# cover-vla/cover-vla

Hardware: AMD Instinct MI355X
Metric: candidate actions scored/sec (whole node), OpenVLA-7B N=32, 224^2 RGB (higher is better)
Workload: dtype bf16; 1 GPU; OpenVLA-7B (DINOv2-L+SigLIP-So400m+Llama-2-7B) N=32 = 8 prompts x 4 samples per GPU, 7 action tokens, 1 224x224 RGB frame(s); CoVer verifier SigLIP2-L/16-384 + 3-member ensemble; random-init weights with decision margins (depth-scaled residual projections, unit-scale embeddings, log-normal gains on the action rows of the head: synth.openvla_state(peaked=True)); candidates_total=32, candidates_per_gpu=32, prompts_per_gpu=8, parallelism=candidate-sharded x1 (weak), own_kv=legacy

## Files before the change

cover_vla_amd/csrc/decode_attn.hip:

```cpp
#include "common.h"
#include "kernels.h"

struct DecAttnDev {
    const bf16_t* qkv; int ld_qkv;
    const float* partial; int n_splits; const float* bias;
    int N, H;
    float scale_log2e;
    const int* positions; const float* cos_t; const float* sin_t; int n_pos, rope_mode;
    const bf16_t* k0; const bf16_t* vt0; int k0_t, k0_h, vt0_h, vt0_d, len0;
    const bf16_t* k1; const bf16_t* vt1; long long k1_slot, vt1_slot; int k1_t, k1_h, vt1_h, vt1_d; const int* slot1; const int* len1; int len1_c;
    bf16_t* k2; bf16_t* vt2; long long k2_slot, vt2_slot; int k2_t, k2_h, vt2_h, vt2_d; const int* slot2; int len2, write_t;
    bf16_t* out; long long o_row;
    int WA, WC;
    int tail_tile;
};

constexpr int DA_NW = 16;

#ifdef COVER_DA_DEBUG
__device__ unsigned long long g_da_dbg[512 * 8];
extern "C" int cover_da_debug(unsigned long long* out) { return (int)hipMemcpyFromSymbol(out, HIP_SYMBOL(g_da_dbg), sizeof(g_da_dbg)); }
#define DAT(slot) do { if (threadIdx.x == 0) g_da_dbg[(((blockIdx.z * gridDim.y + blockIdx.y) * gridDim.x + blockIdx.x) & 511) * 8 + (slot)] = wall_clock64(); } while (0)
__device__ unsigned long long g_da_wave[16 * 8];
extern "C" int cover_da_debug_waves(unsigned long long* out) { return (int)hipMemcpyFromSymbol(out, HIP_SYMBOL(g_da_wave), sizeof(g_da_wave)); }
#define DAW(slot, val) do { if ((threadIdx.x & 63) == 0 && blockIdx.x == 1 && blockIdx.y == 7 && blockIdx.z == 2) g_da_wave[(threadIdx.x >> 6) * 8 + (slot)] = (val); } while (0)
#else
#define DAT(slot) do { } while (0)
#define DAW(slot, val) do { } while (0)
#endif
template <int D, int VS>
__global__ __launch_bounds__(1024) void decode_attn_fused_k(DecAttnDev a) {
    DAT(0);
    DAW(6, wall_clock64());
    constexpr int KS = D / 32, DB = D / 16 / VS, HALF = D / 2, DV = D / VS;
    constexpr int OW = DB * 4 * 64;
    constexpr int IPW = (DB * 4 + DA_NW - 1) / DA_NW;
    static_assert(DB * 4 % DA_NW == 0 || DB * 4 < DA_NW, "merge items must split evenly over the waves");
    __shared__ __attribute__((aligned(16))) bf16_t qs[16 * D];
    __shared__ __attribute__((aligned(16))) bf16_t kn[16 * D];
    __shared__ __attribute__((aligned(16))) bf16_t vn[16 * D];
    __shared__ float so[(DA_NW + 1) * OW];
    __shared__ float sm[(DA_NW + 1) * 16];
    __shared__ float sl[(DA_NW + 1) * 16];
    const int tid = threadIdx.x, lane = tid & 63;
    const int w = __builtin_amdgcn_readfirstlane(tid >> 6);
    const int tile = blockIdx.x, h = blockIdx.y;
    const int dv0 = blockIdx.z * DV;
    const int r = lane & 15, g = lane >> 4;
    const int ncols = 3 * a.H * D;
    const int WB = DA_NW - a.WA - a.WC;

    const int cand_r = tile * 16 + r;
    const bool q_ok = cand_r < a.N;
    const int my_slot1 = q_ok ? (a.slot1 ? a.slot1[cand_r] : cand_r) : -1;
    const int my_len1 = q_ok ? (a.len1 ? a.len1[cand_r] : a.len1_c) : 0;
    const bool p1 = tid < 16 * HALF;
    const int pc = tid / HALF, pi = tid - pc * HALF;
    const int pcand = tile * 16 + pc;
    const bool p1_ok = p1 && pcand < a.N;
    int ppos = 0, pslot2 = pcand;
    if (p1_ok) {
        if (a.rope_mode != 0) ppos = a.positions[pcand];
        if (a.slot2) pslot2 = a.slot2[pcand];
    }
#ifdef COVER_DA_DEBUG
    asm volatile("s_waitcnt vmcnt(0)" ::: "memory");
#endif
    DAT(4);
    float x[6] = {0.f, 0.f, 0.f, 0.f, 0.f, 0.f};
    float cs = 1.f, sn = 0.f;
    if (p1_ok) {
        unsigned col[6];
#pragma unroll
        for (int j = 0; j < 3; ++j) {
            col[2 * j] = (unsigned)((j * a.H + h) * D + pi);
            col[2 * j + 1] = col[2 * j] + HALF;
        }
        float pv[6][4], bs[6] = {0.f, 0.f, 0.f, 0.f, 0.f, 0.f};
        const unsigned pstride = (unsigned)a.N * (unsigned)ncols;
        if (a.n_splits <= 0) {
            const unsigned ro = (unsigned)pcand * (unsigned)a.ld_qkv;
#pragma unroll
            for (int j = 0; j < 6; ++j) x[j] = bf2f(a.qkv[ro + col[j]]);
        } else {
            const unsigned ro = (unsigned)pcand * (unsigned)ncols;
#pragma unroll
            for (int sidx = 0; sidx < 4; ++sidx) {
                if (sidx < a.n_splits) {
                    const float* ps = a.partial + (size_t)sidx * pstride;
#pragma unroll
                    for (int j = 0; j < 6; ++j) pv[j][sidx] = ps[ro + col[j]];
                } else {
#pragma unroll
                    for (int j = 0; j < 6; ++j) pv[j][sidx] = 0.f;
                }
            }
            if (a.bias) {
#pragma unroll
                for (int j = 0; j < 6; ++j) bs[j] = a.bias[col[j]];
            }
        }
        if (a.rope_mode != 0) {
            ppos = ppos < 0 ? 0 : (ppos >= a.n_pos ? a.n_pos - 1 : ppos);
            const unsigned po = (unsigned)(ppos * HALF + pi);
            cs = a.cos_t[po];
            sn = a.sin_t[po];
        }
        if (a.n_splits > 0) {
            const unsigned ro = (unsigned)pcand * (unsigned)ncols;
#pragma unroll
            for (int j = 0; j < 6; ++j) {
                float v = 0.f;
#pragma unroll
                for (int sidx = 0; sidx < 4; ++sidx) v += sidx < a.n_splits ? pv[j][sidx] : 0.f;
                for (int sidx = 4; sidx < a.n_splits; ++sidx) v += a.partial[(size_t)sidx * pstride + ro + col[j]];
                if (a.bias) v += bs[j];
                x[j] = bfround(v);
            }
        }
    }

    asm volatile("s_waitcnt vmcnt(0)" ::: "memory");
    DAT(5);
    bool leader = q_ok;
#pragma unroll
    for (int j = 0; j < 15; ++j) {
        const int other = __shfl(my_slot1, (lane & 48) | j);
        leader = leader && !(j < r && other == my_slot1);
    }
    const unsigned leaders = (unsigned)(__ballot(leader && g == 0) & 0xffffull);
    const int role = w < a.WA ? 0 : (w < a.WA + WB ? 1 : 2);
    const int wl = role == 0 ? w : (role == 1 ? w - a.WA : w - a.WA - WB);
    const int cl = 4 * wl;

    const bf16_t* kbase = nullptr;
    const bf16_t* vbase = nullptr;
    unsigned ko0 = 0, ko1 = 0;
    unsigned vo = 0;
    unsigned vstep = 0;
    unsigned vmask = 0;
    int it = -1, bcol = -1, bslot = 0, blen = 0;
    bool tail_pending = (VS >= 2 && role == 2 && wl == 0 && a.tail_tile >= 0), is_tail = false;
    auto next_tile = [&]() -> bool {
        if (role == 0) {
            it = it < 0 ? wl : it + a.WA;
            const int t0 = 32 * it;
            if (t0 >= a.len0 || it == a.tail_tile) return false;
            int key0 = t0 + 8 * (r >> 2) + (r & 3), key1 = key0 + 4;
            key0 = key0 < a.len0 ? key0 : a.len0 - 1;
            key1 = key1 < a.len0 ? key1 : a.len0 - 1;
            kbase = a.k0 + h * a.k0_h;
            ko0 = key0 * a.k0_t + g * 8;
            ko1 = key1 * a.k0_t + g * 8;
            vbase = a.vt0 + h * a.vt0_h + t0;
            vo = r * a.vt0_d + g * 8;
            vstep = 16 * a.vt0_d;
            vmask = 0;
#pragma unroll
            for (int e = 0; e < 8; ++e) vmask |= (q_ok && t0 + 8 * g + e < a.len0) ? (1u << e) : 0u;
            return true;
        }
        if (role == 1) {
            ++it;
            if (bcol < 0 || 32 * it >= blen) {
                it = 0;
                bool found = false;
                for (int c = bcol + 1; c < 16 && !found; ++c) {
                    if (!((leaders >> c) & 1u)) continue;
                    if (__popc(leaders & ((1u << c) - 1u)) % WB != wl) continue;
                    const int glen = __shfl(my_len1, c);
                    if (glen <= 0) continue;
                    bcol = c; bslot = __builtin_amdgcn_readfirstlane(__shfl(my_slot1, c)); blen = __builtin_amdgcn_readfirstlane(glen);
                    found = true;
                }
                if (!found) return false;
            }
            const int t0 = 32 * it;
            int key0 = t0 + 8 * (r >> 2) + (r & 3), key1 = key0 + 4;
            key0 = key0 < blen ? key0 : blen - 1;
            key1 = key1 < blen ? key1 : blen - 1;
            kbase = a.k1 + (long long)bslot * a.k1_slot + h * a.k1_h;
            ko0 = key0 * a.k1_t + g * 8;
            ko1 = key1 * a.k1_t + g * 8;
            vbase = a.vt1 + (long long)bslot * a.vt1_slot + h * a.vt1_h + t0;
            vo = r * a.vt1_d + g * 8;
            vstep = 16 * a.vt1_d;
            vmask = 0;
#pragma unroll
            for (int e = 0; e < 8; ++e) vmask |= (q_ok && my_slot1 == bslot && t0 + 8 * g + e < blen) ? (1u << e) : 0u;
            return true;
        }
        ++it;
        const int tb = 8 * it;
        if (tb >= a.len2) {
            if (VS < 2 || !tail_pending) return false;
            tail_pending = false;
            is_tail = true;
            const int t0 = 32 * a.tail_tile;
            int key0 = t0 + 8 * (r >> 2) + (r & 3), key1 = key0 + 4;
            key0 = key0 < a.len0 ? key0 : a.len0 - 1;
            key1 = key1 < a.len0 ? key1 : a.len0 - 1;
            kbase = a.k0 + h * a.k0_h;
            ko0 = key0 * a.k0_t + g * 8;
            ko1 = key1 * a.k0_t + g * 8;
            vbase = a.vt0 + h * a.vt0_h + t0;
            vo = r * a.vt0_d + g * 8;
            vstep = 16 * a.vt0_d;
            vmask = 0;
#pragma unroll
            for (int e = 0; e < 8; ++e) vmask |= (q_ok && t0 + 8 * g + e < a.len0) ? (1u << e) : 0u;
            return true;
        }
        int cg = tile * 16 + cl + (r >> 2), cv = tile * 16 + cl + g;
        cg = cg < a.N ? cg : a.N - 1;
        cv = cv < a.N ? cv : a.N - 1;
        const int sk = a.slot2 ? a.slot2[cg] : cg, sv = a.slot2 ? a.slot2[cv] : cv;
        int ta = tb + (r & 3), tc = ta + 4;
        ta = ta < a.len2 ? ta : a.len2 - 1;
        tc = tc < a.len2 ? tc : a.len2 - 1;
        kbase = a.k2 + h * a.k2_h;
        ko0 = (unsigned)sk * (unsigned)a.k2_slot + ta * a.k2_t + g * 8;
        ko1 = (unsigned)sk * (unsigned)a.k2_slot + tc * a.k2_t + g * 8;
        vbase = a.vt2 + h * a.vt2_h + tb;
        vo = (unsigned)sv * (unsigned)a.vt2_slot + r * a.vt2_d;
        vstep = 16 * a.vt2_d;
        vmask = 0;
#pragma unroll
        for (int e = 0; e < 8; ++e) vmask |= (q_ok && cl + g == r && tb + e < a.len2) ? (1u << e) : 0u;
        return true;
    };
    u32x4 kr0[KS], kr1[KS], vr[DB];
    auto load_tile = [&]() {
#pragma unroll
        for (int ks = 0; ks < KS; ++ks) {
            kr0[ks] = *(const u32x4*)(kbase + ko0 + ks * 32);
            kr1[ks] = *(const u32x4*)(kbase + ko1 + ks * 32);
        }
#pragma unroll
        for (int db = 0; db < DB; ++db) vr[db] = *(const u32x4*)(vbase + vo + (db + (dv0 >> 4)) * vstep);
    };
    if (p1) {
        if (p1_ok) {
            if (a.rope_mode == 2) {
                cs = bfround(cs); sn = bfround(sn);
                const float a1 = bfround(bfround(x[0] * cs) + bfround(-x[1] * sn)), a2 = bfround(bfround(x[1] * cs) + bfround(x[0] * sn));
                const float b1 = bfround(bfround(x[2] * cs) + bfround(-x[3] * sn)), b2 = bfround(bfround(x[3] * cs) + bfround(x[2] * sn));
                x[0] = a1; x[1] = a2; x[2] = b1; x[3] = b2;
            } else if (a.rope_mode != 0) {
#pragma clang fp contract(off)
                const float a1 = x[0] * cs - x[1] * sn, a2 = x[1] * cs + x[0] * sn;
                const float b1 = x[2] * cs - x[3] * sn, b2 = x[3] * cs + x[2] * sn;
                x[0] = a1; x[1] = a2; x[2] = b1; x[3] = b2;
            }
        }
        qs[pc * D + pi] = f2bf(x[0]);
        qs[pc * D + pi + HALF] = f2bf(x[1]);
        kn[pc * D + pi] = f2bf(x[2]);
        kn[pc * D + pi + HALF] = f2bf(x[3]);
        vn[pc * D + pi] = f2bf(x[4]);
        vn[pc * D + pi + HALF] = f2bf(x[5]);
    }
    DAT(6);
    bool have = next_tile();
    if (have) load_tile();
    DAW(0, wall_clock64());
    DAW(4, (unsigned long long)role);
    asm volatile("s_waitcnt lgkmcnt(0)\n\ts_barrier" ::: "memory");
    DAT(1);
    DAW(1, wall_clock64());
    if (p1_ok) {
        bf16_t* kd = a.k2 + a.write_t * a.k2_t + h * a.k2_h;
        const unsigned kof = (unsigned)pslot2 * (unsigned)a.k2_slot + pi;
        if (blockIdx.z == 0) { kd[kof] = f2bf(x[2]); kd[kof + HALF] = f2bf(x[3]); }
        bf16_t* vd = a.vt2 + h * a.vt2_h + a.write_t;
        const unsigned vof = (unsigned)pslot2 * (unsigned)a.vt2_slot + pi * a.vt2_d;
        if (pi >= dv0 && pi < dv0 + DV) vd[vof] = f2bf(x[4]);
        if (pi + HALF >= dv0 && pi + HALF < dv0 + DV) vd[vof + HALF * a.vt2_d] = f2bf(x[5]);
    }

    bool first = true;
#ifdef COVER_DA_DEBUG
    int dbg_tiles = 0;
#endif
    int sw = w;
#pragma clang loop unroll(disable)
    while (have) {
        if (VS >= 2 && is_tail && sw == w) {
            if (first) {
#pragma unroll
                for (int i = 0; i < DB * 4; ++i) so[w * OW + i * 64 + lane] = 0.f;
                if (g == 0) {
                    sm[w * 16 + r] = -INFINITY;
                    sl[w * 16 + r] = 0.f;
                }
            }
            sw = DA_NW;
            first = true;
        }
        if (role == 2 && !is_tail) {
            const int e = a.write_t - 8 * it;
            if (e >= 0 && e < 8) {
                const bf16_t* kp = kn + (cl + (r >> 2)) * D + g * 8;
                const bool mine = (r & 3) == (e & 3);
#pragma unroll
                for (int ks = 0; ks < KS; ++ks) {
                    const u32x4 nk = *(const u32x4*)(kp + ks * 32);
                    kr0[ks] = (mine && e < 4) ? nk : kr0[ks];
                    kr1[ks] = (mine && e >= 4) ? nk : kr1[ks];
                    asm volatile("" ::: "memory");
                }
                const unsigned keep = (e & 1) ? 0x0000ffffu : 0xffff0000u;
                const int sh = (e & 1) ? 16 : 0, wi = e >> 1;
#pragma unroll
                for (int db = 0; db < DB; ++db) {
                    const unsigned nv = (unsigned)vn[(cl + g) * D + dv0 + db * 16 + r] << sh;
#pragma unroll
                    for (int q = 0; q < 4; ++q) vr[db][q] = (q == wi) ? ((vr[db][q] & keep) | nv) : vr[db][q];
                    asm volatile("" ::: "memory");
                }
            }
        }
        f32x4 s0 = (f32x4){0.f, 0.f, 0.f, 0.f}, s1 = s0;
#pragma unroll
        for (int ks = 0; ks < KS; ++ks) {
            const bf16x8 qf = as_bf16x8(*(const uint4*)(qs + r * D + ks * 32 + g * 8));
            s0 = __builtin_amdgcn_mfma_f32_16x16x32_bf16(__builtin_bit_cast(bf16x8, kr0[ks]), qf, s0, 0, 0, 0);
            s1 = __builtin_amdgcn_mfma_f32_16x16x32_bf16(__builtin_bit_cast(bf16x8, kr1[ks]), qf, s1, 0, 0, 0);
        }
        float sc[8], m = -INFINITY;
#pragma unroll
        for (int e = 0; e < 8; ++e) {
            sc[e] = ((vmask >> e) & 1u) ? (e < 4 ? s0[e] : s1[e - 4]) * a.scale_log2e : -INFINITY;
            m = fmaxf(m, sc[e]);
        }
        m = fmaxf(m, __shfl_xor(m, 16));
        m = fmaxf(m, __shfl_xor(m, 32));
        float l = 0.f, p[8];
#pragma unroll
        for (int e = 0; e < 8; ++e) {
            p[e] = (m == -INFINITY) ? 0.f : exp2f(sc[e] - m);
            l += p[e];
        }
        l += __shfl_xor(l, 16);
        l += __shfl_xor(l, 32);
        uint4 pp;
        pp.x = pack_bf2(p[0], p[1]); pp.y = pack_bf2(p[2], p[3]); pp.z = pack_bf2(p[4], p[5]); pp.w = pack_bf2(p[6], p[7]);
        const bf16x8 pf = as_bf16x8(pp);
        float* slot = so + sw * OW + lane;
        float fo = 0.f, ft = 1.f;
        if (!first) {
            const float mo = sm[sw * 16 + r], lo = sl[sw * 16 + r];
            const float mx = fmaxf(mo, m);
            fo = (mo == -INFINITY) ? 0.f : exp2f(mo - mx);
            ft = (m == -INFINITY) ? 0.f : exp2f(m - mx);
            m = mx;
            l = lo * fo + l * ft;
        }
#pragma unroll
        for (int db = 0; db < DB; ++db) {
            const f32x4 o = __builtin_amdgcn_mfma_f32_16x16x32_bf16(__builtin_bit_cast(bf16x8, vr[db]), pf, (f32x4){0.f, 0.f, 0.f, 0.f}, 0, 0, 0);
#pragma unroll
            for (int e = 0; e < 4; ++e) {
                float* sp = slot + (db * 4 + e) * 64;
                *sp = first ? o[e] : *sp * fo + o[e] * ft;
            }
            asm volatile("" ::: "memory");
        }
        if (g == 0) {
            sm[sw * 16 + r] = m;
            sl[sw * 16 + r] = l;
        }
#ifdef COVER_DA_DEBUG
        if (first) DAW(2, wall_clock64());
        dbg_tiles++;
#endif
        first = false;
        have = next_tile();
        if (have) load_tile();
    }
#ifdef COVER_DA_DEBUG
    DAW(3, wall_clock64());
    DAW(5, (unsigned long long)dbg_tiles);
#endif
    if (first && sw == w) {
#pragma unroll
        for (int i = 0; i < DB * 4; ++i) so[w * OW + i * 64 + lane] = 0.f;
        if (g == 0) {
            sm[w * 16 + r] = -INFINITY;
            sl[w * 16 + r] = 0.f;
        }
    }
    if (role == 2 && wl == 0 && sw == w) {
#pragma unroll
        for (int i = 0; i < DB * 4; ++i) so[DA_NW * OW + i * 64 + lane] = 0.f;
        if (g == 0) {
            sm[DA_NW * 16 + r] = -INFINITY;
            sl[DA_NW * 16 + r] = 0.f;
        }
    }

    asm volatile("s_waitcnt lgkmcnt(0)\n\ts_barrier" ::: "memory");
    DAT(2);
    if (!q_ok) return;
    float mx = -INFINITY;
#pragma unroll
    for (int i = 0; i < DA_NW + 1; ++i) mx = fmaxf(mx, sm[i * 16 + r]);
    float lt = 0.f, f[DA_NW + 1];
#pragma unroll
    for (int i = 0; i < DA_NW + 1; ++i) {
        const float mi = sm[i * 16 + r];
        f[i] = (mi == -INFINITY) ? 0.f : exp2f(mi - mx);
        lt += sl[i * 16 + r] * f[i];
    }
    const float inv = lt > 0.f ? 1.f / lt : 0.f;
    const int item0 = w * IPW, db = item0 >> 2, e0 = item0 & 3;
    if (item0 >= DB * 4) return;
    float o[IPW];
#pragma unroll
    for (int e = 0; e < IPW; ++e) {
        float acc = 0.f;
#pragma unroll
        for (int i = 0; i < DA_NW + 1; ++i) acc += so[i * OW + (item0 + e) * 64 + lane] * f[i];
        o[e] = acc * inv;
    }
    bf16_t* op = a.out + (long long)cand_r * a.o_row + (long long)h * D + dv0 + db * 16 + 4 * g + e0;
    if constexpr (IPW == 2) {
        *(uint32_t*)op = pack_bf2(o[0], o[1]);
    } else {
        *op = f2bf(o[0]);
    }
    DAT(3);
}

hipError_t launch_decode_attention_fused(const cover_decode_attn_args* x, hipStream_t st) {
    if (x->N <= 0) return hipSuccess;
    if (x->D != 64 && x->D != 128) return hipErrorInvalidValue;
    for (int i = 0; i < 3; ++i)
        if (x->seg[i].mask_mode != COVER_MASK_LEN) return hipErrorInvalidValue;
    if (x->seg[0].len <= 0 || x->seg[2].len <= 0 || x->write_t < 0 || x->write_t >= x->seg[2].len) return hipErrorInvalidValue;
    if (x->rope_mode != 0 && (!x->cos_table || !x->sin_table || !x->positions)) return hipErrorInvalidValue;
    DecAttnDev a;
    a.qkv = (const bf16_t*)x->qkv; a.ld_qkv = x->ld_qkv;
    a.partial = x->partial; a.n_splits = x->n_splits; a.bias = x->bias;
    a.N = x->N; a.H = x->H;
    a.scale_log2e = x->scale * 1.4426950408889634f;
    a.positions = x->positions; a.cos_t = x->cos_table; a.sin_t = x->sin_table; a.n_pos = x->n_pos; a.rope_mode = x->rope_mode;
    const cover_kv_segment &s0 = x->seg[0], &s1 = x->seg[1], &s2 = x->seg[2];
    const long long slot0 = 0;
    a.k0 = (const bf16_t*)s0.k + slot0 * s0.k_slot_stride; a.vt0 = (const bf16_t*)s0.vt + slot0 * s0.vt_slot_stride;
    const long long strides[] = {s0.k_t_stride, s0.k_h_stride, s0.vt_h_stride, s0.vt_d_stride, s1.k_t_stride, s1.k_h_stride, s1.vt_h_stride,
                                 s1.vt_d_stride, s2.k_t_stride, s2.k_h_stride, s2.vt_h_stride, s2.vt_d_stride};
    for (long long v : strides)
        if (v < 0 || v > (1ll << 26)) return hipErrorInvalidValue;
    if ((long long)x->N * 3 * x->H * x->D * (x->n_splits > 0 ? x->n_splits : 1) >= (1ll << 31)) return hipErrorInvalidValue;
    if (!s2.slot_of_batch && ((long long)x->N * s2.k_slot_stride >= (1ll << 31) || (long long)x->N * s2.vt_slot_stride >= (1ll << 31)))
        return hipErrorInvalidValue;
    if ((s2.vt_d_stride & 7) || (s0.vt_d_stride & 7) || (s1.vt_d_stride & 7)) return hipErrorInvalidValue;
    a.k0_t = (int)s0.k_t_stride; a.k0_h = (int)s0.k_h_stride; a.vt0_h = (int)s0.vt_h_stride; a.vt0_d = (int)s0.vt_d_stride; a.len0 = s0.len;
    a.k1 = (const bf16_t*)s1.k; a.vt1 = (const bf16_t*)s1.vt;
    a.k1_slot = s1.k_slot_stride; a.k1_t = (int)s1.k_t_stride; a.k1_h = (int)s1.k_h_stride;
    a.vt1_slot = s1.vt_slot_stride; a.vt1_h = (int)s1.vt_h_stride; a.vt1_d = (int)s1.vt_d_stride;
    a.slot1 = s1.slot_of_batch; a.len1 = s1.len_of_batch; a.len1_c = s1.len;
    a.k2 = (bf16_t*)s2.k; a.vt2 = (bf16_t*)s2.vt;
    a.k2_slot = s2.k_slot_stride; a.k2_t = (int)s2.k_t_stride; a.k2_h = (int)s2.k_h_stride;
    a.vt2_slot = s2.vt_slot_stride; a.vt2_h = (int)s2.vt_h_stride; a.vt2_d = (int)s2.vt_d_stride;
    a.slot2 = s2.slot_of_batch; a.len2 = s2.len; a.write_t = x->write_t;
    a.out = (bf16_t*)x->out; a.o_row = x->out_row_stride;
    const int nA = (s0.len + 31) / 32;
    a.WC = 4;
    a.WA = nA < 9 ? nA : 9;
    a.tail_tile = -1;
    static const char* vs_env = getenv("COVER_DA_VSPLIT");
    const int units = ((x->N + 15) / 16) * x->H;
    int VS = vs_env ? (atoi(vs_env) == 4 ? 4 : atoi(vs_env) == 2 ? 2 : 1) : (units <= 64 ? 4 : units <= 128 ? 2 : 1);
    if (x->D != 128 && VS == 4) VS = 2;
    static const char* tail_env = getenv("COVER_DA_TAIL");
    if (nA == 9 && VS >= 2 && !(tail_env && tail_env[0] == '0')) { a.WA = 8; a.tail_tile = 8; }
    dim3 grid((x->N + 15) / 16, x->H, VS), block(64 * DA_NW);
    const int pid = prof_enabled() ? prof_open(st, 2, 0.0) : -1;
    if (x->D == 128) {
        if (VS == 4) hipLaunchKernelGGL((decode_attn_fused_k<128, 4>), grid, block, 0, st, a);
        else if (VS == 2) hipLaunchKernelGGL((decode_attn_fused_k<128, 2>), grid, block, 0, st, a);
        else hipLaunchKernelGGL((decode_attn_fused_k<128, 1>), grid, block, 0, st, a);
    } else {
        if (VS == 2) hipLaunchKernelGGL((decode_attn_fused_k<64, 2>), grid, block, 0, st, a);
        else hipLaunchKernelGGL((decode_attn_fused_k<64, 1>), grid, block, 0, st, a);
    }
    prof_close(st, pid);
    return hipGetLastError();
}
```

Measured before the change: 956.8 candidates/s.

## Move decode-attn QKV prologue onto C-role waves with vector loads and priority

The QKV prologue (sum split-K partials, add bias, apply RoPE, stage q/k/v into LDS and write the new K/V to cache) now runs on the four C-role waves, each lane handling several contiguous elements with vectorized float4/uint2 loads and stores. Before, every thread in the first half of the block did one scalar element. Those waves also raise their scheduling priority until the barrier, so the prologue that gates the barrier finishes sooner while the other waves prefetch their K/V tiles. An optional late-prefetch variant is compiled in but off. The wide path needs pointer and stride alignment checks, falls back otherwise, and doubles the template instantiations.

```diff
diff --git a/cover_vla_amd/csrc/decode_attn.hip b/cover_vla_amd/csrc/decode_attn.hip
--- a/cover_vla_amd/csrc/decode_attn.hip
+++ b/cover_vla_amd/csrc/decode_attn.hip
@@ -20,19 +20,45 @@
 #ifdef COVER_DA_DEBUG
 __device__ unsigned long long g_da_dbg[512 * 8];
 extern "C" int cover_da_debug(unsigned long long* out) { return (int)hipMemcpyFromSymbol(out, HIP_SYMBOL(g_da_dbg), sizeof(g_da_dbg)); }
-#define DAT(slot) do { if (threadIdx.x == 0) g_da_dbg[(((blockIdx.z * gridDim.y + blockIdx.y) * gridDim.x + blockIdx.x) & 511) * 8 + (slot)] = wall_clock64(); } while (0)
+#define DAT_IF(cond, slot) do { if (cond) g_da_dbg[(((blockIdx.z * gridDim.y + blockIdx.y) * gridDim.x + blockIdx.x) & 511) * 8 + (slot)] = wall_clock64(); } while (0)
+#define DAT(slot) DAT_IF(threadIdx.x == 0, slot)
 __device__ unsigned long long g_da_wave[16 * 8];
 extern "C" int cover_da_debug_waves(unsigned long long* out) { return (int)hipMemcpyFromSymbol(out, HIP_SYMBOL(g_da_wave), sizeof(g_da_wave)); }
 #define DAW(slot, val) do { if ((threadIdx.x & 63) == 0 && blockIdx.x == 1 && blockIdx.y == 7 && blockIdx.z == 2) g_da_wave[(threadIdx.x >> 6) * 8 + (slot)] = (val); } while (0)
 #else
+#define DAT_IF(cond, slot) do { } while (0)
 #define DAT(slot) do { } while (0)
 #define DAW(slot, val) do { } while (0)
 #endif
-template <int D, int VS>
+#ifndef COVER_DA_P1_PRIO
+#define COVER_DA_P1_PRIO 1
+#endif
+#ifndef COVER_DA_AB_LATE
+#define COVER_DA_AB_LATE 0
+#endif
+
+template <int n> __device__ __forceinline__ void ld_f32(const float* p, float (&o)[n]) {
+    if constexpr (n == 4) { const float4 v = *(const float4*)p; o[0] = v.x; o[1] = v.y; o[2] = v.z; o[3] = v.w; }
+    else if constexpr (n == 2) { const float2 v = *(const float2*)p; o[0] = v.x; o[1] = v.y; }
+    else o[0] = *p;
+}
+template <int n> __device__ __forceinline__ void ld_bf16(const bf16_t* p, bf16_t (&o)[n]) {
+    if constexpr (n == 4) { const uint2 v = *(const uint2*)p; o[0] = (bf16_t)v.x; o[1] = (bf16_t)(v.x >> 16); o[2] = (bf16_t)v.y; o[3] = (bf16_t)(v.y >> 16); }
+    else if constexpr (n == 2) { const uint32_t v = *(const uint32_t*)p; o[0] = (bf16_t)v; o[1] = (bf16_t)(v >> 16); }
+    else o[0] = *p;
+}
+template <int n> __device__ __forceinline__ void st_bf16(bf16_t* p, const float (&x)[n]) {
+    if constexpr (n == 4) { uint2 v; v.x = pack_bf2(x[0], x[1]); v.y = pack_bf2(x[2], x[3]); *(uint2*)p = v; }
+    else if constexpr (n == 2) *(uint32_t*)p = pack_bf2(x[0], x[1]);
+    else *p = f2bf(x[0]);
+}
+
+template <int D, int VS, bool P1V>
 __global__ __launch_bounds__(1024) void decode_attn_fused_k(DecAttnDev a) {
     DAT(0);
     DAW(6, wall_clock64());
     constexpr int KS = D / 32, DB = D / 16 / VS, HALF = D / 2, DV = D / VS;
+    constexpr int PPL = P1V ? HALF / 16 : 1;
     constexpr int OW = DB * 4 * 64;
     constexpr int IPW = (DB * 4 + DA_NW - 1) / DA_NW;
     static_assert(DB * 4 % DA_NW == 0 || DB * 4 < DA_NW, "merge items must split evenly over the waves");
@@ -54,8 +80,17 @@
     const bool q_ok = cand_r < a.N;
     const int my_slot1 = q_ok ? (a.slot1 ? a.slot1[cand_r] : cand_r) : -1;
     const int my_len1 = q_ok ? (a.len1 ? a.len1[cand_r] : a.len1_c) : 0;
-    const bool p1 = tid < 16 * HALF;
-    const int pc = tid / HALF, pi = tid - pc * HALF;
+    const int role = w < a.WA ? 0 : (w < a.WA + WB ? 1 : 2);
+    const int wl = role == 0 ? w : (role == 1 ? w - a.WA : w - a.WA - WB);
+    const int cl = 4 * wl;
+#if COVER_DA_P1_PRIO
+    if constexpr (P1V) {
+        if (role == 2) __builtin_amdgcn_s_setprio(3);
+    }
+#endif
+    const bool p1 = P1V ? role == 2 : tid < 16 * HALF;
+    const int pc = P1V ? cl + g : tid / HALF, pi = P1V ? r * PPL : tid - pc * HALF;
+    const bool p1_stamp = P1V ? (role == 2 && wl == 0 && lane == 0) : tid == 0;
     const int pcand = tile * 16 + pc;
     const bool p1_ok = p1 && pcand < a.N;
     int ppos = 0, pslot2 = pcand;
@@ -66,9 +101,15 @@
 #ifdef COVER_DA_DEBUG
     asm volatile("s_waitcnt vmcnt(0)" ::: "memory");
 #endif
-    DAT(4);
-    float x[6] = {0.f, 0.f, 0.f, 0.f, 0.f, 0.f};
-    float cs = 1.f, sn = 0.f;
+    DAT_IF(p1_stamp, 4);
+    float x[6][PPL];
+    float cs[PPL], sn[PPL];
+#pragma unroll
+    for (int e = 0; e < PPL; ++e) {
+#pragma unroll
+        for (int j = 0; j < 6; ++j) x[j][e] = 0.f;
+        cs[e] = 1.f; sn[e] = 0.f;
+    }
     if (p1_ok) {
         unsigned col[6];
 #pragma unroll
@@ -76,52 +117,83 @@
             col[2 * j] = (unsigned)((j * a.H + h) * D + pi);
             col[2 * j + 1] = col[2 * j] + HALF;
         }
-        float pv[6][4], bs[6] = {0.f, 0.f, 0.f, 0.f, 0.f, 0.f};
         const unsigned pstride = (unsigned)a.N * (unsigned)ncols;
+        auto load_cos_sin = [&]() {
+            if (a.rope_mode != 0) {
+                ppos = ppos < 0 ? 0 : (ppos >= a.n_pos ? a.n_pos - 1 : ppos);
+                const unsigned po = (unsigned)(ppos * HALF + pi);
+                ld_f32<PPL>(a.cos_t + po, cs);
+                ld_f32<PPL>(a.sin_t + po, sn);
+            }
+        };
         if (a.n_splits <= 0) {
             const unsigned ro = (unsigned)pcand * (unsigned)a.ld_qkv;
 #pragma unroll
-            for (int j = 0; j < 6; ++j) x[j] = bf2f(a.qkv[ro + col[j]]);
+            for (int j = 0; j < 6; ++j) {
+                bf16_t raw[PPL];
+                ld_bf16<PPL>(a.qkv + ro + col[j], raw);
+#pragma unroll
+                for (int e = 0; e < PPL; ++e) x[j][e] = bf2f(raw[e]);
+            }
+            load_cos_sin();
         } else {
             const unsigned ro = (unsigned)pcand * (unsigned)ncols;
-#pragma unroll
-            for (int sidx = 0; sidx < 4; ++sidx) {
+            constexpr int NSL = PPL == 4 ? 2 : 4;
+            float pv[6][NSL][PPL], bs[6][PPL];
+#pragma unroll
+            for (int sidx = 0; sidx < NSL; ++sidx) {
                 if (sidx < a.n_splits) {
                     const float* ps = a.partial + (size_t)sidx * pstride;
 #pragma unroll
-                    for (int j = 0; j < 6; ++j) pv[j][sidx] = ps[ro + col[j]];
+                    for (int j = 0; j < 6; ++j) ld_f32<PPL>(ps + ro + col[j], pv[j][sidx]);
                 } else {
 #pragma unroll
-                    for (int j = 0; j < 6; ++j) pv[j][sidx] = 0.f;
-                }
-            }
-            if (a.bias) {
-#pragma unroll
-                for (int j = 0; j < 6; ++j) bs[j] = a.bias[col[j]];
-            }
-        }
-        if (a.rope_mode != 0) {
-            ppos = ppos < 0 ? 0 : (ppos >= a.n_pos ? a.n_pos - 1 : ppos);
-            const unsigned po = (unsigned)(ppos * HALF + pi);
-            cs = a.cos_t[po];
-            sn = a.sin_t[po];
-        }
-        if (a.n_splits > 0) {
-            const unsigned ro = (unsigned)pcand * (unsigned)ncols;
+                    for (int j = 0; j < 6; ++j)
+#pragma unroll
+                        for (int e = 0; e < PPL; ++e) pv[j][sidx][e] = 0.f;
+                }
+            }
 #pragma unroll
             for (int j = 0; j < 6; ++j) {
-                float v = 0.f;
-#pragma unroll
-                for (int sidx = 0; sidx < 4; ++sidx) v += sidx < a.n_splits ? pv[j][sidx] : 0.f;
-                for (int sidx = 4; sidx < a.n_splits; ++sidx) v += a.partial[(size_t)sidx * pstride + ro + col[j]];
-                if (a.bias) v += bs[j];
-                x[j] = bfround(v);
-            }
+                if (a.bias) {
+                    ld_f32<PPL>(a.bias + col[j], bs[j]);
+                } else {
+#pragma unroll
+                    for (int e = 0; e < PPL; ++e) bs[j][e] = 0.f;
+                }
+            }
+            load_cos_sin();
+            float v[6][PPL];
+#pragma unroll
+            for (int j = 0; j < 6; ++j)
+#pragma unroll
+                for (int e = 0; e < PPL; ++e) {
+                    v[j][e] = 0.f;
+#pragma unroll
+                    for (int sidx = 0; sidx < NSL; ++sidx) v[j][e] += sidx < a.n_splits ? pv[j][sidx][e] : 0.f;
+                }
+            for (int sidx = NSL; sidx < a.n_splits; ++sidx) {
+                const float* ps = a.partial + (size_t)sidx * pstride;
+                float t[6][PPL];
+#pragma unroll
+                for (int j = 0; j < 6; ++j) ld_f32<PPL>(ps + ro + col[j], t[j]);
+#pragma unroll
+                for (int j = 0; j < 6; ++j)
+#pragma unroll
+                    for (int e = 0; e < PPL; ++e) v[j][e] += t[j][e];
+            }
+#pragma unroll
+            for (int j = 0; j < 6; ++j)
+#pragma unroll
+                for (int e = 0; e < PPL; ++e) {
+                    if (a.bias) v[j][e] += bs[j][e];
+                    x[j][e] = bfround(v[j][e]);
+                }
         }
     }
 
     asm volatile("s_waitcnt vmcnt(0)" ::: "memory");
-    DAT(5);
+    DAT_IF(p1_stamp, 5);
     bool leader = q_ok;
 #pragma unroll
     for (int j = 0; j < 15; ++j) {
@@ -129,9 +201,6 @@
         leader = leader && !(j < r && other == my_slot1);
     }
     const unsigned leaders = (unsigned)(__ballot(leader && g == 0) & 0xffffull);
-    const int role = w < a.WA ? 0 : (w < a.WA + WB ? 1 : 2);
-    const int wl = role == 0 ? w : (role == 1 ? w - a.WA : w - a.WA - WB);
-    const int cl = 4 * wl;
 
     const bf16_t* kbase = nullptr;
     const bf16_t* vbase = nullptr;
@@ -242,40 +311,63 @@
     if (p1) {
         if (p1_ok) {
             if (a.rope_mode == 2) {
-                cs = bfround(cs); sn = bfround(sn);
-                const float a1 = bfround(bfround(x[0] * cs) + bfround(-x[1] * sn)), a2 = bfround(bfround(x[1] * cs) + bfround(x[0] * sn));
-                const float b1 = bfround(bfround(x[2] * cs) + bfround(-x[3] * sn)), b2 = bfround(bfround(x[3] * cs) + bfround(x[2] * sn));
-                x[0] = a1; x[1] = a2; x[2] = b1; x[3] = b2;
+#pragma unroll
+                for (int e = 0; e < PPL; ++e) {
+                    const float c = bfround(cs[e]), s = bfround(sn[e]);
+                    const float a1 = bfround(bfround(x[0][e] * c) + bfround(-x[1][e] * s)), a2 = bfround(bfround(x[1][e] * c) + bfround(x[0][e] * s));
+                    const float b1 = bfround(bfround(x[2][e] * c) + bfround(-x[3][e] * s)), b2 = bfround(bfround(x[3][e] * c) + bfround(x[2][e] * s));
+                    x[0][e] = a1; x[1][e] = a2; x[2][e] = b1; x[3][e] = b2;
+                }
             } else if (a.rope_mode != 0) {
 #pragma clang fp contract(off)
-                const float a1 = x[0] * cs - x[1] * sn, a2 = x[1] * cs + x[0] * sn;
-                const float b1 = x[2] * cs - x[3] * sn, b2 = x[3] * cs + x[2] * sn;
-                x[0] = a1; x[1] = a2; x[2] = b1; x[3] = b2;
-            }
-        }
-        qs[pc * D + pi] = f2bf(x[0]);
-        qs[pc * D + pi + HALF] = f2bf(x[1]);
-        kn[pc * D + pi] = f2bf(x[2]);
-        kn[pc * D + pi + HALF] = f2bf(x[3]);
-        vn[pc * D + pi] = f2bf(x[4]);
-        vn[pc * D + pi + HALF] = f2bf(x[5]);
-    }
-    DAT(6);
-    bool have = next_tile();
-    if (have) load_tile();
+#pragma unroll
+                for (int e = 0; e < PPL; ++e) {
+                    const float c = cs[e], s = sn[e];
+                    const float a1 = x[0][e] * c - x[1][e] * s, a2 = x[1][e] * c + x[0][e] * s;
+                    const float b1 = x[2][e] * c - x[3][e] * s, b2 = x[3][e] * c + x[2][e] * s;
+                    x[0][e] = a1; x[1][e] = a2; x[2][e] = b1; x[3][e] = b2;
+                }
+            }
+        }
+        st_bf16<PPL>(qs + pc * D + pi, x[0]);
+        st_bf16<PPL>(qs + pc * D + pi + HALF, x[1]);
+        st_bf16<PPL>(kn + pc * D + pi, x[2]);
+        st_bf16<PPL>(kn + pc * D + pi + HALF, x[3]);
+        st_bf16<PPL>(vn + pc * D + pi, x[4]);
+        st_bf16<PPL>(vn + pc * D + pi + HALF, x[5]);
+    }
+    DAT_IF(p1_stamp, 6);
+    constexpr bool AB_LATE = P1V && COVER_DA_AB_LATE;
+    bool have = false;
+    if (!AB_LATE || role == 2) {
+        have = next_tile();
+        if (have) load_tile();
+    }
     DAW(0, wall_clock64());
     DAW(4, (unsigned long long)role);
     asm volatile("s_waitcnt lgkmcnt(0)\n\ts_barrier" ::: "memory");
     DAT(1);
     DAW(1, wall_clock64());
+#if COVER_DA_P1_PRIO
+    if constexpr (P1V) {
+        if (role == 2) __builtin_amdgcn_s_setprio(0);
+    }
+#endif
+    if (AB_LATE && role != 2) {
+        have = next_tile();
+        if (have) load_tile();
+    }
     if (p1_ok) {
         bf16_t* kd = a.k2 + a.write_t * a.k2_t + h * a.k2_h;
         const unsigned kof = (unsigned)pslot2 * (unsigned)a.k2_slot + pi;
-        if (blockIdx.z == 0) { kd[kof] = f2bf(x[2]); kd[kof + HALF] = f2bf(x[3]); }
+        if (blockIdx.z == 0) { st_bf16<PPL>(kd + kof, x[2]); st_bf16<PPL>(kd + kof + HALF, x[3]); }
         bf16_t* vd = a.vt2 + h * a.vt2_h + a.write_t;
         const unsigned vof = (unsigned)pslot2 * (unsigned)a.vt2_slot + pi * a.vt2_d;
-        if (pi >= dv0 && pi < dv0 + DV) vd[vof] = f2bf(x[4]);
-        if (pi + HALF >= dv0 && pi + HALF < dv0 + DV) vd[vof + HALF * a.vt2_d] = f2bf(x[5]);
+#pragma unroll
+        for (int e = 0; e < PPL; ++e) {
+            if (pi + e >= dv0 && pi + e < dv0 + DV) vd[vof + e * a.vt2_d] = f2bf(x[4][e]);
+            if (pi + e + HALF >= dv0 && pi + e + HALF < dv0 + DV) vd[vof + (e + HALF) * a.vt2_d] = f2bf(x[5][e]);
+        }
     }
 
     bool first = true;
@@ -430,6 +522,18 @@
         *op = f2bf(o[0]);
     }
     DAT(3);
+}
+
+template <bool P1V>
+static void launch_da(int D, int VS, dim3 grid, dim3 block, hipStream_t st, const DecAttnDev& a) {
+    if (D == 128) {
+        if (VS == 4) hipLaunchKernelGGL((decode_attn_fused_k<128, 4, P1V>), grid, block, 0, st, a);
+        else if (VS == 2) hipLaunchKernelGGL((decode_attn_fused_k<128, 2, P1V>), grid, block, 0, st, a);
+        else hipLaunchKernelGGL((decode_attn_fused_k<128, 1, P1V>), grid, block, 0, st, a);
+    } else {
+        if (VS == 2) hipLaunchKernelGGL((decode_attn_fused_k<64, 2, P1V>), grid, block, 0, st, a);
+        else hipLaunchKernelGGL((decode_attn_fused_k<64, 1, P1V>), grid, block, 0, st, a);
+    }
 }
 
 hipError_t launch_decode_attention_fused(const cover_decode_attn_args* x, hipStream_t st) {
@@ -476,16 +580,17 @@
     if (x->D != 128 && VS == 4) VS = 2;
     static const char* tail_env = getenv("COVER_DA_TAIL");
     if (nA == 9 && VS >= 2 && !(tail_env && tail_env[0] == '0')) { a.WA = 8; a.tail_tile = 8; }
+    const char* p1_env = getenv("COVER_DA_P1");
+    const int run = x->D / 32;
+    auto aligned = [](const void* p, size_t bytes) { return ((uintptr_t)p & (bytes - 1)) == 0; };
+    const bool wide_ok = a.WC == 4 && aligned(a.partial, 4 * run) && aligned(a.bias, 4 * run) && aligned(a.cos_t, 4 * run) && aligned(a.sin_t, 4 * run) &&
+                         aligned(a.qkv, 2 * run) && a.ld_qkv % run == 0 && aligned(a.k2, 2 * run) && a.k2_slot % run == 0 && a.k2_t % run == 0 &&
+                         a.k2_h % run == 0;
+    const bool p1v = wide_ok && !(p1_env && p1_env[0] == '0');
     dim3 grid((x->N + 15) / 16, x->H, VS), block(64 * DA_NW);
     const int pid = prof_enabled() ? prof_open(st, 2, 0.0) : -1;
-    if (x->D == 128) {
-        if (VS == 4) hipLaunchKernelGGL((decode_attn_fused_k<128, 4>), grid, block, 0, st, a);
-        else if (VS == 2) hipLaunchKernelGGL((decode_attn_fused_k<128, 2>), grid, block, 0, st, a);
-        else hipLaunchKernelGGL((decode_attn_fused_k<128, 1>), grid, block, 0, st, a);
-    } else {
-        if (VS == 2) hipLaunchKernelGGL((decode_attn_fused_k<64, 2>), grid, block, 0, st, a);
-        else hipLaunchKernelGGL((decode_attn_fused_k<64, 1>), grid, block, 0, st, a);
-    }
+    if (p1v) launch_da<true>(x->D, VS, grid, block, st, a);
+    else launch_da<false>(x->D, VS, grid, block, st, a);
     prof_close(st, pid);
     return hipGetLastError();
 }
```

Result: no change. 955.3 candidates/s (-0.2%).
